# Rafae1130/qwen_inference_engine

Measured on AMD Instinct MI355X. Metric: decode tokens/s + prefill tok/s, Qwen2-7B bf16 batch=1, 1/2/4/8 MI355X, higher is better.
Workload: dtype bf16; 1 GPU; Qwen2-7B bf16 decode, batch=1, prompt=2048, gen=512; batch_per_gpu=1, batch=1, prompt=2048, gen=512, parallelism=single, graph=True, kv=contiguous

## Files before the change

include/qie/qie_engine.h:

```cpp
#ifndef QIE_ENGINE_H
#define QIE_ENGINE_H

#include "qie_types.h"
#include "qie_ops.h"

#ifdef __cplusplus
extern "C" {
#endif

typedef struct qie_engine qie_engine;
typedef struct qie_comm qie_comm;
typedef struct qie_batch qie_batch;
typedef struct qie_index qie_index;

int qie_index_load_meta(const char* meta_data_txt, qie_index** out);
int qie_index_synthetic(const qie_model_spec* spec, qie_index** out);
int qie_index_count(const qie_index* idx);
int qie_index_get(const qie_index* idx, int i, const char** name, const char** short_name,
                  int32_t* layer, int64_t* off0, int64_t* off1, int32_t* ndim, int64_t* shape4);
int64_t qie_index_total_bytes(const qie_index* idx);
int qie_index_write_meta(const qie_index* idx, const char* path);
void qie_index_destroy(qie_index* idx);

#define QIE_COMM_ID_BYTES 128
// ... 3 lines not shown
#define QIE_COMM_PEER_HANDLE_BYTES 128
int qie_comm_create_peer(int32_t world, int32_t rank, int32_t device, qie_comm** out, void* handle_out);
int qie_comm_peer_connect(qie_comm* c, const void* handles);
int qie_comm_create_peer_local(int32_t world, qie_comm** out);
int qie_comm_peer_error(const qie_comm* c, int32_t* err);
int qie_comm_peer_set_mode(qie_comm* c, int32_t tagged, int32_t push);
int qie_comm_allreduce_residual_bf16(qie_comm* c, const float* part, void* x, int64_t n, void* stream);
int qie_comm_time_exchange(qie_comm* c, const float* part, void* x, int64_t n, int32_t count, int32_t reps,
                           int32_t form, void* stream, float* us_out);
int qie_comm_rank(const qie_comm* c, int32_t* world, int32_t* rank);
int qie_comm_allreduce_sum_f32(qie_comm* c, float* buf, int64_t n, void* stream);
int qie_comm_allreduce_max_u64(qie_comm* c, uint64_t* buf, int64_t n, void* stream);
void qie_comm_destroy(qie_comm* c);

typedef struct qie_engine_opts {
    int32_t device;
    int32_t max_ctx;
    int32_t use_graph;
    int32_t tp_rank, tp_size;
    void* tp_comm;
    int32_t weight_fp8;
    int32_t comm_always;
    int32_t prefill_fp8;
    int32_t reserved[5];
} qie_engine_opts;

int qie_engine_create(const qie_model_spec* spec, const qie_engine_opts* opts, qie_engine** out);
int qie_engine_init_synthetic(qie_engine* e, uint64_t seed, float w_scale, float norm_scale,
                              float bias_scale);
int qie_engine_load_weights_bin(qie_engine* e, const char* weights_bin, const char* meta_data_txt,
                                int64_t chunk_bytes);
int qie_engine_set_weights(qie_engine* e, const qie_model_weights* w);
int qie_engine_weights(const qie_engine* e, qie_model_weights* out, const qie_layer_weights** layers);
int qie_engine_spec(const qie_engine* e, qie_model_spec* out);
void* qie_engine_stream(qie_engine* e);
int qie_engine_sync(qie_engine* e);
void qie_engine_destroy(qie_engine* e);

int qie_batch_create(qie_engine* e, int32_t batch, int32_t max_ctx, qie_batch** out);
void qie_batch_destroy(qie_batch* b);

int qie_batch_create_paged(qie_engine* e, int32_t batch, int32_t max_ctx, int32_t page_tokens,
                           int32_t n_pages, qie_batch** out);
int qie_batch_release(qie_batch* b, int32_t seq);
int qie_batch_page_stats(qie_batch* b, int32_t* free_pages, int32_t* pages_per_seq, int32_t* page_tokens);
int qie_batch_block_table(qie_batch* b, int32_t seq, int32_t* host_pages, int32_t n);

int qie_prefill(qie_batch* b, int32_t seq, const int32_t* ids, int32_t n, const qie_sampling* s,
                int32_t* next_id);
int qie_prefill_batch(qie_batch* b, int32_t seq0, int32_t n_seqs, const int32_t* ids, int32_t len,
                      const qie_sampling* s, int32_t* next_ids);
int qie_prefill_append(qie_batch* b, int32_t seq, const int32_t* ids, int32_t n, int32_t pos0,
                       const qie_sampling* s, int32_t* next_id);
int qie_decode_step(qie_batch* b, const qie_sampling* s, int32_t* next_ids);
int qie_decode(qie_batch* b, int32_t n_steps, const qie_sampling* s, int32_t* out_ids);
int qie_batch_logits(qie_batch* b, void* host_out);
int qie_batch_positions(qie_batch* b, int32_t* host_pos);
int qie_batch_history(qie_batch* b, int32_t seq, int32_t* host_ids, int32_t n);
int qie_batch_set_position(qie_batch* b, int32_t seq, int32_t pos, int32_t token);
int qie_batch_set_decode_mode(qie_batch* b, int32_t mode);
int qie_batch_decode_mode(const qie_batch* b);
int qie_batch_pk_trace(qie_batch* b, int32_t enable, uint64_t* host_out, int64_t n);
int qie_batch_dims(const qie_batch* b, int32_t* batch, int32_t* max_ctx);
int qie_batch_kv_cache(const qie_batch* b, int32_t seq, qie_kv_cache* out);
int qie_batch_reserve(qie_batch* b, int32_t seq, int32_t n_tokens);
int qie_engine_arena(const qie_engine* e, void** base, int64_t* bytes);
int qie_engine_rope_tables(const qie_engine* e, const float** rope_cos, const float** rope_sin,
                           int32_t* rows);
int qie_batch_time_kernel(qie_batch* b, int32_t which, int32_t iters, double* avg_us,
                          double* bytes);
int qie_batch_debug_step(qie_batch* b, const qie_sampling* smp, int32_t* next_ids, void* host_x);

#ifdef __cplusplus
}
#endif

#endif
```

qwen_inference_engine_amd/_lib.py:

```python
from __future__ import annotations

import ctypes as C
import os

_HERE = os.path.dirname(os.path.abspath(__file__))
LIB_PATH = os.environ.get("QIE_LIB") or os.path.join(_HERE, "lib", "libqie.so")

QIE_NUMERICS_REF = 0
QIE_NUMERICS_HF = 1
QIE_EPI_STORE = 0
QIE_EPI_RESIDUAL = 1
QIE_EPI_SWIGLU = 2
QIE_EPI_F32 = 3
QIE_LINEAR_FP8 = 1
QIE_LINEAR_TILE256 = 2
QIE_LINEAR_TILE128 = 4
QIE_LINEAR_STREAMK = 8
QIE_LINEAR_FP8_T16 = 16
QIE_LINEAR_ACT_FP8 = 32
QIE_ATTN_PREROPED = 0x100
QIE_COMM_ID_BYTES = 128
QIE_COMM_PEER_HANDLE_BYTES = 128


# ... 97 lines not shown
    ("qie_keys_to_ids", C.c_int, [_P, _I64, _P, _P]),
    ("qie_tensor_id", C.c_uint32, [C.c_char_p]),
    ("qie_synthetic_fill", C.c_int, [_P, _I64, _U32, _U64, _F, _F, _P]),
    ("qie_synthetic_fill_host", C.c_int, [_P, _I64, _U32, _U64, _F, _F]),
    ("qie_synthetic_fill_slice", C.c_int, [_P, _I64, _I64, _I64, _I64, _I64, _U32, _U64, _F, _F, _P]),
    ("qie_scale_rows_pow2", C.c_int, [_P, _I64, _I64, _I64, _I64, _I32, _P]),
    ("qie_fp8_weight_bytes", C.c_int64, [_I64, _I64]),
    ("qie_quantize_fp8", C.c_int, [_P, _I64, _I64, _P, _P]),
    ("qie_quantize_rows_fp8", C.c_int, [_P, _I64, _I64, _I64, _P, _I64, _P, _P]),
    ("qie_quantize_fp8_host", C.c_int, [_P, _I64, _I64, _P]),
    ("qie_dequantize_fp8", C.c_int, [_P, _I64, _I64, _P, _P]),
    ("qie_fp8_tile16", C.c_int, [_P, _I64, _I64, _P, _P]),
    ("qie_debug_fp8_decode", C.c_int, [_P]),
    ("qie_debug_fp8_decode_bf16", C.c_int, [_P]),
    ("qie_comm_unique_id", C.c_int, [_P]),
    ("qie_comm_create_rccl", C.c_int, [_P, _I32, _I32, _I32, C.POINTER(_P)]),
    ("qie_comm_create_local", C.c_int, [_I32, C.POINTER(_P)]),
    ("qie_comm_create_peer", C.c_int, [_I32, _I32, _I32, C.POINTER(_P), _P]),
    ("qie_comm_peer_connect", C.c_int, [_P, _P]),
    ("qie_comm_create_peer_local", C.c_int, [_I32, C.POINTER(_P)]),
    ("qie_comm_peer_error", C.c_int, [_P, _PI32]),
    ("qie_comm_allreduce_residual_bf16", C.c_int, [_P, _P, _P, _I64, _P]),
    ("qie_comm_peer_set_mode", C.c_int, [_P, _I32, _I32]),
    ("qie_comm_time_exchange", C.c_int, [_P, _P, _P, _I64, _I32, _I32, _I32, _P, C.POINTER(C.c_float)]),
    ("qie_comm_rank", C.c_int, [_P, _PI32, _PI32]),
    ("qie_comm_allreduce_sum_f32", C.c_int, [_P, _P, _I64, _P]),
    ("qie_comm_allreduce_max_u64", C.c_int, [_P, _P, _I64, _P]),
    ("qie_comm_destroy", None, [_P]),
    ("qie_index_load_meta", C.c_int, [C.c_char_p, C.POINTER(_P)]),
    ("qie_index_synthetic", C.c_int, [C.POINTER(ModelSpecC), C.POINTER(_P)]),
    ("qie_index_count", C.c_int, [_P]),
    ("qie_index_get", C.c_int, [_P, C.c_int, _PCC, _PCC, _PI32, _PI64, _PI64, _PI32, _PI64]),
    ("qie_index_total_bytes", C.c_int64, [_P]),
    ("qie_index_write_meta", C.c_int, [_P, C.c_char_p]),
    ("qie_index_destroy", None, [_P]),
    ("qie_engine_create", C.c_int, [C.POINTER(ModelSpecC), C.POINTER(EngineOptsC), C.POINTER(_P)]),
    ("qie_engine_init_synthetic", C.c_int, [_P, _U64, _F, _F, _F]),
    ("qie_engine_load_weights_bin", C.c_int, [_P, C.c_char_p, C.c_char_p, _I64]),
    ("qie_engine_set_weights", C.c_int, [_P, C.POINTER(ModelWeightsC)]),
    ("qie_engine_weights", C.c_int, [_P, C.POINTER(ModelWeightsC), C.POINTER(C.POINTER(LayerWeightsC))]),
    ("qie_engine_spec", C.c_int, [_P, C.POINTER(ModelSpecC)]),
    ("qie_engine_stream", _P, [_P]),
    ("qie_engine_sync", C.c_int, [_P]),
    ("qie_engine_destroy", None, [_P]),
    ("qie_batch_create", C.c_int, [_P, _I32, _I32, C.POINTER(_P)]),
    ("qie_batch_destroy", None, [_P]),
    ("qie_batch_create_paged", C.c_int, [_P, _I32, _I32, _I32, _I32, C.POINTER(_P)]),
    ("qie_batch_release", C.c_int, [_P, _I32]),
    ("qie_batch_page_stats", C.c_int, [_P, _PI32, _PI32, _PI32]),
    ("qie_batch_block_table", C.c_int, [_P, _I32, _PI32, _I32]),
    ("qie_prefill", C.c_int, [_P, _I32, _PI32, _I32, C.POINTER(SamplingC), _PI32]),
    ("qie_prefill_batch", C.c_int, [_P, _I32, _I32, _PI32, _I32, C.POINTER(SamplingC), _PI32]),
    ("qie_prefill_append", C.c_int, [_P, _I32, _PI32, _I32, _I32, C.POINTER(SamplingC), _PI32]),
    ("qie_decode_step", C.c_int, [_P, C.POINTER(SamplingC), _PI32]),
    ("qie_decode", C.c_int, [_P, _I32, C.POINTER(SamplingC), _PI32]),
    ("qie_batch_logits", C.c_int, [_P, _P]),
    ("qie_batch_positions", C.c_int, [_P, _PI32]),
    ("qie_batch_history", C.c_int, [_P, _I32, _PI32, _I32]),
    ("qie_batch_set_position", C.c_int, [_P, _I32, _I32, _I32]),
    ("qie_batch_dims", C.c_int, [_P, _PI32, _PI32]),
    ("qie_batch_set_decode_mode", C.c_int, [_P, _I32]),
    ("qie_batch_decode_mode", C.c_int, [_P]),
    ("qie_batch_pk_trace", C.c_int, [_P, _I32, _P, C.c_int64]),
    ("qie_batch_kv_cache", C.c_int, [_P, _I32, C.POINTER(KvCacheC)]),
    ("qie_batch_reserve", C.c_int, [_P, _I32, _I32]),
    ("qie_engine_arena", C.c_int, [_P, C.POINTER(_P), _PI64]),
    ("qie_engine_rope_tables", C.c_int, [_P, C.POINTER(_P), C.POINTER(_P), _PI32]),
    ("qie_batch_time_kernel", C.c_int, [_P, _I32, _I32, _PD, _PD]),
    ("qie_batch_debug_step", C.c_int, [_P, _P, _PI32, _P]),
]

_lib = None


class QieError(RuntimeError):
    pass


def load(path: str = LIB_PATH):
    global _lib
    if _lib is not None:
        return _lib
    if not os.path.exists(path):
        raise QieError(f"{path} not built; run __graft_entry__.build() or make -C "
                       f"qwen_inference_engine_amd/csrc")
    lib = C.CDLL(path)
    for name, res, args in SIGNATURES:
        fn = getattr(lib, name)
        fn.restype = res
        fn.argtypes = args
    _lib = lib
    return lib


def check(rc: int, what: str = "") -> None:
    if rc != 0:
        msg = _lib.qie_last_error().decode() if _lib is not None else ""
        raise QieError(f"{what} failed (rc={rc}): {msg}")
```

qwen_inference_engine_amd/csrc/engine.hip:

```cpp
#include "qie_common.hpp"
#include "linear_plan.hpp"
#include "../../include/qie/qie_engine.h"
#include "qie_index.hpp"
#include "qie_comm.hpp"

#include <chrono>
#include <cstring>
#include <fstream>
#include <vector>

namespace qie {
bool dec8_applies(const qie_linear_args* a);
int dec8_reserve(hipStream_t st);
bool persist_supported(const qie_model_spec& s, int B, int tp, bool fp8, bool paged, int ncu, const char** why);
size_t persist_attn_table_bytes(int n_layers);
int persist_attn_table(const qie_model_spec& s, const qie_layer_weights* h_layers, const void* qkv_scratch,
                       const int32_t* pos, const float* rope_cos, const float* rope_sin, const qie_kv_cache* cache,
                       void* dec_ws, void* d_attp, hipStream_t st);
int persist_decode_launch(const qie_model_spec& s, const qie_layer_weights* d_layers, const void* d_attp,
                          uint16_t* x_res, unsigned long long* granules, const unsigned* epoch, unsigned* err,
                          const int32_t* pos, int splits_target, unsigned long long* ts, hipStream_t st);
int64_t persist_granule_count(const qie_model_spec& s);
int persist_ts_slots();
}
// ... 540 lines not shown
    if (e->fp8_t16_head) a.flags |= QIE_LINEAR_FP8_T16;
    a.x = x; a.ldx = ldx;
    a.w[0] = e->w.lm_head; a.seg_rows[0] = Vl;
    a.M = M; a.K = s.hidden; a.N = Vl;
    a.y = b->logits + (int64_t)m0 * Vl; a.ldy = Vl;
    a.epilogue = QIE_EPI_STORE;
    a.norm_w = e->w.final_norm; a.norm_eps = s.rms_eps; a.numerics = s.numerics;
    QIE_TRY(prenorm(b, a, M));
    const bool greedy = is_greedy(smp);
    if (greedy) {
        a.argmax_keys = (uint64_t*)(b->d_keys + m0);
        a.key_col0 = e->sh.vocab0;
    }
    QIE_TRY(linear(&a, LinearExtras{}, st));
    if (greedy && use_comm(e)) QIE_TRY(e->comm->allreduce_max_u64((uint64_t*)(b->d_keys + m0), M, st));
    if (!greedy) {
        const uint16_t* lg = b->logits + (int64_t)m0 * Vl;
        if (use_comm(e)) {
            QIE_TRY(gather_logits(b, m0, M));
            lg = b->logits_full + (int64_t)m0 * s.vocab;
        }
        QIE_TRY(qie_sample(lg, M, s.vocab, s.vocab, smp, b->d_step + m0, b->d_ids + m0, b->samp_ws, st));
    }
    hipLaunchKernelGGL(finalize_kernel, dim3(M), dim3(256), 0, st, m0, greedy ? b->d_keys : nullptr,
                       b->d_ids, b->d_ids, b->d_pos, b->d_step, b->d_hist, b->max_ctx,
                       (const uint4*)e->w.embed, (uint4*)b->x_res, (int64_t)s.hidden / 8, s.vocab, rope_cur_args(b),
                       b->pk_mem ? pk_epoch_ptr(b) : nullptr);
    QIE_LAUNCH_CHECK();
    return 0;
}

static bool pk_on(const qie_batch* b) { return b->decode_mode == 1 && b->pk_mem && !b->dbg_x; }

static int pk_splits_target(const qie_batch* b) { (void)b; return 32; }

static int enqueue_layers_persistent(qie_batch* b) {
    qie_engine* e = b->e;
    return persist_decode_launch(e->spec, b->d_layers, b->d_attp, b->x_res, (unsigned long long*)b->pk_mem,
                                 pk_epoch_ptr(b), pk_epoch_ptr(b) + 1, b->d_pos, pk_splits_target(b), b->pk_ts,
                                 e->stream);
}

static int enqueue_decode(qie_batch* b, const qie_sampling* smp) {
    if (pk_on(b)) QIE_TRY(enqueue_layers_persistent(b));
    else
        for (int l = 0; l < b->e->spec.n_layers; l++) QIE_TRY(enqueue_layer_decode(b, l));
    return enqueue_head(b, b->x_res, b->e->spec.hidden, 0, b->B, smp);
}

static bool prefill_mx(const qie_engine* e) {
    return e->fp8 && e->opts.prefill_fp8;
}

static int64_t prefill_attn_ws_bytes(const qie_batch* b, int64_t n, bool extend) {
    const qie_model_spec& s = b->e->spec;
    if (extend) return qie_attention_extend_workspace_bytes(n, b->e->sh.nq, s.head_dim, b->max_ctx + b->run_pad);
    return qie_attention_workspace_bytes(n, b->e->sh.nq, s.head_dim, b->max_ctx);
}

static int ensure_prefill_scratch(qie_batch* b, int64_t n, bool extend) {
    if (n <= b->pf_rows) {
        const int64_t ws = prefill_attn_ws_bytes(b, n, extend);
        if (ws > b->pf_attn_ws_bytes) {
            hipFree(b->pf_attn_ws);
            b->pf_attn_ws = nullptr;
            b->pf_attn_ws_bytes = 0;
            QIE_TRY(dmalloc(&b->pf_attn_ws, (size_t)ws));
            b->pf_attn_ws_bytes = ws;
        }
        return 0;
    }
    const qie_model_spec& s = b->e->spec;
    const TpShard& sh = b->e->sh;
    const int64_t H = s.hidden, QD = (int64_t)sh.nq * s.head_dim, KD = (int64_t)sh.nkv * s.head_dim;
    void** olds[] = {(void**)&b->pf_x, (void**)&b->pf_hn, (void**)&b->pf_qkv, (void**)&b->pf_q, (void**)&b->pf_att,
                     (void**)&b->pf_h, (void**)&b->pf_pos, (void**)&b->pf_ids, &b->pf_attn_ws, (void**)&b->pf_part,
                     (void**)&b->pf_q8, (void**)&b->pf_e8};
    for (void** p : olds) {
        if (*p) hipFree(*p);
        *p = nullptr;
    }
    b->pf_rows = 0;
    if (use_comm(b->e)) QIE_TRY(dmalloc((void**)&b->pf_part, n * H * 4));
    QIE_TRY(dmalloc((void**)&b->pf_x, n * H * 2));
    QIE_TRY(dmalloc((void**)&b->pf_hn, n * H * 2));
    QIE_TRY(dmalloc((void**)&b->pf_qkv, n * (QD + 2 * KD) * 2));
    QIE_TRY(dmalloc((void**)&b->pf_q, n * QD * 2));
    QIE_TRY(dmalloc((void**)&b->pf_att, n * QD * 2));
    QIE_TRY(dmalloc((void**)&b->pf_h, n * (int64_t)sh.ffn * 2));
    if (prefill_mx(b->e)) {
        const int64_t kmax = std::max<int64_t>(std::max<int64_t>(H, QD), sh.ffn);
        QIE_TRY(dmalloc((void**)&b->pf_q8, n * kmax));
        QIE_TRY(dmalloc((void**)&b->pf_e8, std::max<int64_t>(n, 16)));
    }
    QIE_TRY(dmalloc((void**)&b->pf_pos, n * 4));
    QIE_TRY(dmalloc((void**)&b->pf_ids, n * 4));
    b->pf_attn_ws = nullptr;
    b->pf_attn_ws_bytes = 0;
    int64_t ws = prefill_attn_ws_bytes(b, n, extend);
    QIE_TRY(dmalloc(&b->pf_attn_ws, (size_t)ws));
    b->pf_attn_ws_bytes = ws;
    b->pf_rows = n;
    return 0;
}

static int pk_fail(unsigned w) {
    return fail(-8, "decode: the persistent decode step gave up on a hand-off wait (error word 0x%x: a CU never "
                    "published its part within the bound); outputs of this step are invalid", w);
}
static int pk_check(qie_batch* b) {
    if (!b->pk_mem) return 0;
    unsigned w = 0;
    QIE_HIP(hipMemcpyAsync(&w, pk_epoch_ptr(b) + 1, 4, hipMemcpyDeviceToHost, b->e->stream));
    QIE_HIP(hipStreamSynchronize(b->e->stream));
    return w ? pk_fail(w) : 0;
}

static int sync_ids(qie_batch* b, int32_t* next_ids) {
    if (!next_ids) return pk_check(b);
    qie_engine* e = b->e;
    QIE_HIP(hipMemcpyAsync(next_ids, b->d_ids, b->B * 4, hipMemcpyDeviceToHost, e->stream));
    const unsigned* ew = use_comm(e) ? e->comm->error_word() : nullptr;
    unsigned err = 0, pkw = 0;
    if (ew) QIE_HIP(hipMemcpyAsync(&err, ew, sizeof(err), hipMemcpyDeviceToHost, e->stream));
    if (b->pk_mem) QIE_HIP(hipMemcpyAsync(&pkw, pk_epoch_ptr(b) + 1, 4, hipMemcpyDeviceToHost, e->stream));
    QIE_HIP(hipStreamSynchronize(e->stream));
    if (pkw) return pk_fail(pkw);
    if (ew) {
        if (err) return fail(-7, "decode: tensor-parallel exchange failed on the device (error word %u: a peer rank "
                                 "did not arrive within the bounded wait); the communicator is unusable", err);
        return 0;
    }
    return comm_check(e, "decode");
}

}

extern "C" {

int qie_engine_create(const qie_model_spec* spec, const qie_engine_opts* opts, qie_engine** out) {
    QIE_REQUIRE(spec && out, "qie_engine_create: bad arguments");
    const qie_model_spec& s = *spec;
    QIE_REQUIRE(s.n_layers > 0 && s.hidden > 0 && s.n_heads > 0 && s.n_kv_heads > 0 && s.head_dim > 0 &&
                    s.ffn > 0 && s.vocab > 0 && s.n_heads % s.n_kv_heads == 0,
                "qie_engine_create: invalid model spec");
    QIE_REQUIRE(s.hidden % 8 == 0 && s.ffn % 8 == 0 && (s.head_dim == 64 || s.head_dim == 128),
                "qie_engine_create: hidden/ffn must be multiples of 8 and head_dim 64 or 128");
    qie_comm* comm = opts ? (qie_comm*)opts->tp_comm : nullptr;
    const int tp = comm ? comm->world : 1;
    TpShard probe;
    QIE_REQUIRE(shard_heads(s.n_heads, s.n_kv_heads, tp, 0, probe) && s.ffn % tp == 0 && (s.ffn / tp) % 8 == 0 &&
                    s.vocab % tp == 0,
// ... 416 lines not shown
    if (page_tokens == 0) page_tokens = 128;
    QIE_REQUIRE(page_tokens >= 128 && (page_tokens & (page_tokens - 1)) == 0,
                "qie_batch_create_paged: page_tokens %d must be a power of two >= 128", page_tokens);
    QIE_REQUIRE(n_pages >= 0, "qie_batch_create_paged: bad n_pages");
    QIE_REQUIRE(n_pages == 0 || n_pages >= 2, "qie_batch_create_paged: need the scratch page and one more");
    return batch_create(e, batch, max_ctx, page_tokens, n_pages, out);
}

int qie_batch_release(qie_batch* b, int32_t seq) {
    QIE_REQUIRE(b && seq >= 0 && seq < b->B, "qie_batch_release: bad arguments");
    drop_pages(b, seq);
    b->idle[seq] = 1;
    QIE_TRY(flush_table(b));
    qie_engine* e = b->e;
    hipLaunchKernelGGL(set_state_kernel, dim3(1), dim3(256), 0, e->stream, seq, 0, 0, 0, b->d_pos, b->d_step, b->d_hist,
                       b->max_ctx, (const uint4*)e->w.embed, (uint4*)b->x_res, (int64_t)e->spec.hidden / 8, 1, rope_cur_args(b));
    QIE_LAUNCH_CHECK();
    QIE_HIP(hipStreamSynchronize(e->stream));
    b->h_pos[seq] = 0;
    return 0;
}

int qie_batch_page_stats(qie_batch* b, int32_t* free_pages, int32_t* pages_per_seq, int32_t* page_tokens) {
    QIE_REQUIRE(b, "qie_batch_page_stats: null batch");
    if (free_pages) *free_pages = (int32_t)b->free_pages.size();
    if (pages_per_seq)
        for (int m = 0; m < b->B; m++) pages_per_seq[m] = b->d_table ? b->held[m] : 0;
    if (page_tokens) *page_tokens = b->page_tokens;
    return 0;
}

int qie_batch_block_table(qie_batch* b, int32_t seq, int32_t* host_pages, int32_t n) {
    QIE_REQUIRE(b && b->d_table && host_pages && seq >= 0 && seq < b->B && n >= 0 && n <= b->max_pages,
                "qie_batch_block_table: bad arguments (paged batch, n <= max_pages)");
    QIE_HIP(hipStreamSynchronize(b->e->stream));
    QIE_HIP(d2h(b->e, host_pages, b->d_table + (int64_t)seq * b->max_pages, (size_t)n * 4));
    return 0;
}

void qie_batch_destroy(qie_batch* b) {
    if (!b) return;
    if (b->e && b->e->stream) hipStreamSynchronize(b->e->stream);
    if (b->gexec) hipGraphExecDestroy(b->gexec);
    void* ps[] = {b->kc, b->vc, b->d_table, b->d_pos, b->d_rope_cur, b->d_step, b->d_hist, b->d_ids, b->d_keys, b->x_res, b->qkv, b->q,
                  b->att, b->h, b->logits, b->attn_ws, b->dec_ws, b->samp_ws, b->pf_x, b->pf_hn, b->pf_qkv, b->pf_q,
                  b->pf_att, b->pf_h, b->pf_pos, b->pf_ids, b->pf_attn_ws, b->part, b->logits_full,
                  b->gather_tmp, b->pf_part, b->xn, b->pf_q8, b->pf_e8, b->pk_mem, b->d_layers, b->d_attp, b->pk_ts};
    for (void* p : ps)
        if (p) hipFree(p);
    delete b;
}

static int prefill_rows(qie_batch* b, int seq0, int n_seqs, const int32_t* ids, int len, int pos0,
                        const qie_sampling* smp, int32_t* next_ids, const char* who) {
    QIE_REQUIRE(b && ids && len > 0 && n_seqs > 0 && seq0 >= 0 && seq0 + n_seqs <= b->B && pos0 >= 0,
                "%s: bad arguments", who);
    QIE_REQUIRE((int64_t)pos0 + len < b->max_ctx, "%s: %d tokens from position %d do not fit max_ctx %d", who, len,
                pos0, b->max_ctx);
    const bool append = pos0 > 0;
    qie_engine* e = b->e;
    const qie_model_spec& s = e->spec;
    if (append) {
        QIE_REQUIRE(n_seqs == 1, "%s: one sequence per call", who);
        QIE_REQUIRE(!b->idle[seq0], "%s: slot %d holds no live sequence", who, seq0);
        QIE_REQUIRE(pos0 <= b->h_pos[seq0], "%s: pos0 %d is past sequence %d's current position %d", who, pos0, seq0,
                    b->h_pos[seq0]);
        QIE_REQUIRE(!(e->fp8 && e->opts.prefill_fp8),
                    "%s: not available on a prefill_fp8 engine (block-scaled fp8 activations are defined for a "
                    "prefill from position 0 only: an append has no reference to be checked against)", who);
    }
    const int64_t n = (int64_t)n_seqs * len;
    QIE_REQUIRE(n <= INT32_MAX, "%s: %lld rows", who, (long long)n);
    for (int64_t i = 0; i < n; i++)
        QIE_REQUIRE(ids[i] >= 0 && ids[i] < s.vocab, "%s: token id %d out of range", who, ids[i]);
    hipStream_t st = e->stream;
    if (append && b->d_table) {
        const int64_t need = ((int64_t)pos0 + len + b->page_tokens - 1) / b->page_tokens - b->held[seq0];
        if (need > (int64_t)b->free_pages.size())
            return fail(-28, "%s: KV pool exhausted (%lld more pages needed for %d rows at position %d, %zu free)",
                        who, (long long)need, len, pos0, b->free_pages.size());
    }
    QIE_TRY(ensure_prefill_scratch(b, n, append));
    if (b->d_table && !append) {
        const int64_t need = ((int64_t)len + b->page_tokens - 1) / b->page_tokens * n_seqs;
        int64_t held = 0;
        for (int z = 0; z < n_seqs; z++) held += b->held[seq0 + z];
        QIE_REQUIRE(need <= (int64_t)b->free_pages.size() + held,
                    "%s: KV pool exhausted (%lld pages needed, %zu free + %lld held by slots %d..%d)", who,
                    (long long)need, b->free_pages.size(), (long long)held, seq0, seq0 + n_seqs - 1);
    }
    if (!append)
        for (int z = 0; z < n_seqs; z++) drop_pages(b, seq0 + z);
    for (int z = 0; z < n_seqs; z++) {
        QIE_TRY(ensure_pages(b, seq0 + z, (int64_t)pos0 + len));
        b->idle[seq0 + z] = 0;
    }
    QIE_TRY(flush_table(b));
    const TpShard& sh = e->sh;
    const int64_t H = s.hidden, hd = s.head_dim, QD = (int64_t)sh.nq * hd, KD = (int64_t)sh.nkv * hd;
    const int64_t QKVD = QD + 2 * KD, I = sh.ffn;
    QIE_HIP(hipMemcpyAsync(b->pf_ids, ids, (size_t)n * 4, hipMemcpyHostToDevice, st));
    hipLaunchKernelGGL(iota_kernel, dim3((unsigned)((n + 255) / 256)), dim3(256), 0, st, b->pf_pos, (int)n, len, pos0);
    hipLaunchKernelGGL(copy_ids_kernel, dim3((len + 255) / 256, n_seqs), dim3(256), 0, st, b->pf_ids,
                       b->d_hist + (int64_t)seq0 * b->max_ctx + pos0, len, (int64_t)b->max_ctx);
    QIE_TRY(qie_embedding(e->w.embed, b->pf_ids, b->pf_x, n, H, st));
    const qie_kv_cache cache = batch_cache(b, seq0);
    const bool pf16 = e->fp8 && !e->layers_pf.empty() && (n >= 256 || (e->fp8_t16 && n > 16));
    auto pf_base = [&]() {
        qie_linear_args a = lin_proj(e);
        if (pf16) a.flags &= ~(QIE_LINEAR_FP8 | QIE_LINEAR_FP8_T16);
        return a;
    };
    const bool mx = prefill_mx(e);
    auto attend = [&](int l) -> int {
        if (append)
            return qie_attention_extend(b->pf_q, n, b->pf_pos, len, &cache, l, sh.nq, b->pf_att, b->pf_attn_ws, st);
        return qie_attention(b->pf_q, n, b->pf_pos, len, &cache, l, sh.nq, b->pf_att, b->pf_attn_ws, st);
    };
    auto mx_in = [&](qie_linear_args& a, const uint16_t* x, int64_t K) -> int {
        QIE_TRY(qie_quantize_rows_fp8(x, K, n, K, b->pf_q8, K, b->pf_e8, st));
        a.x = b->pf_q8; a.ldx = K; a.x_exps = b->pf_e8;
        a.flags |= QIE_LINEAR_ACT_FP8;
        return 0;
    };
    for (int l = 0; l < s.n_layers; l++) {
        if (mx) {
            const qie_layer_weights& L = e->layers[l];
            QIE_TRY(qie_rmsnorm(b->pf_x, L.attn_norm, b->pf_hn, n, H, s.rms_eps, s.numerics, st));
            qie_linear_args a = lin_proj(e);
            QIE_TRY(mx_in(a, b->pf_hn, H));
            a.w[0] = L.wq; a.w[1] = L.wk; a.w[2] = L.wv;
            a.bias[0] = L.bq; a.bias[1] = L.bk; a.bias[2] = L.bv;
            a.seg_rows[0] = QD; a.seg_rows[1] = KD; a.seg_rows[2] = KD;
            a.M = n; a.K = H; a.N = QKVD; a.y = b->pf_qkv; a.ldy = QKVD; a.epilogue = QIE_EPI_STORE;
            QIE_TRY(qie_linear(&a, st));
            QIE_TRY(qie_qkv_post(b->pf_qkv, n, b->pf_pos, len, L.q_norm, L.k_norm, e->rope_cos, e->rope_sin, sh.nq,
                                 &cache, l, s.rms_eps, s.numerics, b->pf_q, st));
            QIE_TRY(attend(l));
            a = lin_proj(e);
            QIE_TRY(mx_in(a, b->pf_att, QD));
            a.w[0] = L.wo; a.seg_rows[0] = H;
            a.M = n; a.K = QD; a.N = H; a.ldy = H;
            QIE_TRY(row_parallel(b, a, b->pf_x, b->pf_part, n));
            QIE_TRY(qie_rmsnorm(b->pf_x, L.ffn_norm, b->pf_hn, n, H, s.rms_eps, s.numerics, st));
            a = lin_proj(e);
            QIE_TRY(mx_in(a, b->pf_hn, H));
            a.w[0] = L.w_gate; a.w[1] = L.w_up; a.seg_rows[0] = I; a.seg_rows[1] = I;
            a.M = n; a.K = H; a.N = I; a.y = b->pf_h; a.ldy = I; a.epilogue = QIE_EPI_SWIGLU;
            QIE_TRY(qie_linear(&a, st));
            a = lin_proj(e);
            QIE_TRY(mx_in(a, b->pf_h, I));
            a.w[0] = L.w_down; a.seg_rows[0] = H;
            a.M = n; a.K = I; a.N = H; a.ldy = H;
            QIE_TRY(row_parallel(b, a, b->pf_x, b->pf_part, n));
            continue;
        }
        const qie_layer_weights& L = pf16 ? e->layers_pf[l] : e->layers[l];
        QIE_TRY(qie_rmsnorm(b->pf_x, L.attn_norm, b->pf_hn, n, H, s.rms_eps, s.numerics, st));
        qie_linear_args a = pf_base();
        a.x = b->pf_hn; a.ldx = H;
        a.w[0] = L.wq; a.w[1] = L.wk; a.w[2] = L.wv;
        a.bias[0] = L.bq; a.bias[1] = L.bk; a.bias[2] = L.bv;
        a.seg_rows[0] = QD; a.seg_rows[1] = KD; a.seg_rows[2] = KD;
        a.M = n; a.K = H; a.N = QKVD; a.y = b->pf_qkv; a.ldy = QKVD; a.epilogue = QIE_EPI_STORE;
        QIE_TRY(qie_linear(&a, st));
        QIE_TRY(qie_qkv_post(b->pf_qkv, n, b->pf_pos, len, L.q_norm, L.k_norm, e->rope_cos, e->rope_sin, sh.nq,
                             &cache, l, s.rms_eps, s.numerics, b->pf_q, st));
        QIE_TRY(attend(l));
        a = pf_base();
        a.x = b->pf_att; a.ldx = QD; a.w[0] = L.wo; a.seg_rows[0] = H;
        a.M = n; a.K = QD; a.N = H; a.ldy = H;
        QIE_TRY(row_parallel(b, a, b->pf_x, b->pf_part, n));
        QIE_TRY(qie_rmsnorm(b->pf_x, L.ffn_norm, b->pf_hn, n, H, s.rms_eps, s.numerics, st));
        a = pf_base();
        a.x = b->pf_hn; a.ldx = H; a.w[0] = L.w_gate; a.w[1] = L.w_up; a.seg_rows[0] = I; a.seg_rows[1] = I;
        a.M = n; a.K = H; a.N = I; a.y = b->pf_h; a.ldy = I; a.epilogue = QIE_EPI_SWIGLU;
        QIE_TRY(qie_linear(&a, st));
        a = pf_base();
        a.x = b->pf_h; a.ldx = I; a.w[0] = L.w_down; a.seg_rows[0] = H;
        a.M = n; a.K = I; a.N = H; a.ldy = H;
        QIE_TRY(row_parallel(b, a, b->pf_x, b->pf_part, n));
    }
    for (int z = 0; z < n_seqs; z++) {
        hipLaunchKernelGGL(set_state_kernel, dim3(1), dim3(64), 0, st, seq0 + z, pos0 + len - 1, 0,
                           ids[(int64_t)z * len + len - 1], b->d_pos, b->d_step, b->d_hist, b->max_ctx,
                           (const uint4*)e->w.embed, (uint4*)b->x_res, (int64_t)H / 8, 0, rope_cur_args(b));
        QIE_LAUNCH_CHECK();
    }
    const uint16_t* last = b->pf_x + (int64_t)(len - 1) * H;
    if (n_seqs > 1) {
        QIE_HIP(hipMemcpy2DAsync(b->pf_hn, (size_t)H * 2, last, (size_t)len * H * 2, (size_t)H * 2, n_seqs,
                                 hipMemcpyDeviceToDevice, st));
        last = b->pf_hn;
    }
    QIE_TRY(enqueue_head(b, last, H, seq0, n_seqs, smp));
    for (int z = 0; z < n_seqs; z++) b->h_pos[seq0 + z] = pos0 + len;
    if (next_ids) {
        QIE_HIP(hipMemcpyAsync(next_ids, b->d_ids + seq0, (size_t)n_seqs * 4, hipMemcpyDeviceToHost, st));
        QIE_HIP(hipStreamSynchronize(st));
        QIE_TRY(comm_check(e, who));
    }
    return 0;
}

int qie_prefill(qie_batch* b, int32_t seq, const int32_t* ids, int32_t n, const qie_sampling* smp, int32_t* next_id) {
    return prefill_rows(b, seq, 1, ids, n, 0, smp, next_id, "qie_prefill");
}

int qie_prefill_append(qie_batch* b, int32_t seq, const int32_t* ids, int32_t n, int32_t pos0,
                       const qie_sampling* smp, int32_t* next_id) {
    QIE_REQUIRE(pos0 >= 1, "qie_prefill_append: pos0 must be >= 1 (a sequence starts with qie_prefill)");
    return prefill_rows(b, seq, 1, ids, n, pos0, smp, next_id, "qie_prefill_append");
}

int qie_prefill_batch(qie_batch* b, int32_t seq0, int32_t n_seqs, const int32_t* ids, int32_t len,
                      const qie_sampling* smp, int32_t* next_ids) {
    return prefill_rows(b, seq0, n_seqs, ids, len, 0, smp, next_ids, "qie_prefill_batch");
}

static bool same_sampling(const qie_sampling& a, const qie_sampling* b) {
    qie_sampling g{1, 0.f, 1.f, 0};
    const qie_sampling& bb = b ? *b : g;
    return a.top_k == bb.top_k && a.temperature == bb.temperature && a.top_p == bb.top_p && a.seed == bb.seed;
}

static int launch_step(qie_batch* b, const qie_sampling* smp) {
    qie_engine* e = b->e;
    if (!e->opts.use_graph) return enqueue_decode(b, smp);
    if (!b->graph_ok || !same_sampling(b->gs, smp)) {
        if (b->gexec) hipGraphExecDestroy(b->gexec);
        b->gexec = nullptr;
        b->graph_ok = false;
        hipGraph_t g = nullptr;
        QIE_HIP(hipStreamBeginCapture(e->stream, hipStreamCaptureModeThreadLocal));
        int rc = enqueue_decode(b, smp);
        hipError_t he = hipStreamEndCapture(e->stream, &g);
        if (rc) {
            if (g) hipGraphDestroy(g);
            return rc;
        }
        if (he != hipSuccess) return fail((int)he, "graph capture: %s", hipGetErrorString(he));
        if (dev_env("QIE_GRAPH_DUMP", 0)) {
            size_t n = 0;
            hipGraphGetNodes(g, nullptr, &n);
            std::vector<hipGraphNode_t> nodes(n);
            hipGraphGetNodes(g, nodes.data(), &n);
            size_t max_shm = 0;
            for (size_t i = 0; i < n; i++) {
                hipGraphNodeType t;
                hipGraphNodeGetType(nodes[i], &t);
                if (t == hipGraphNodeTypeKernel) {
                    hipKernelNodeParams kp{};
                    hipGraphKernelNodeGetParams(nodes[i], &kp);
                    max_shm = std::max(max_shm, (size_t)kp.sharedMemBytes);
                    fprintf(stderr, "graph node %zu: kernel %p grid %u,%u,%u block %u,%u,%u dyn_lds %u\n", i, kp.func,
                            kp.gridDim.x, kp.gridDim.y, kp.gridDim.z, kp.blockDim.x, kp.blockDim.y, kp.blockDim.z,
                            kp.sharedMemBytes);
                } else {
                    fprintf(stderr, "graph node %zu: type %d\n", i, (int)t);
                }
            }
            fprintf(stderr, "graph: %zu nodes, max dynamic LDS %zu B\n", n, max_shm);
        }
        he = hipGraphInstantiate(&b->gexec, g, nullptr, nullptr, 0);
        hipGraphDestroy(g);
// ... 389 lines not shown
```

qwen_inference_engine_amd/engine.py:

```python
from __future__ import annotations

import ctypes as C
import dataclasses
from typing import Dict, List, Optional, Sequence

import numpy as np

from . import _lib
from .spec import ModelSpec
from .weights import SynthParams

REF_PREFILL_SAMPLING = dict(top_k=50, temperature=1.0, seed=1234)
REF_DECODE_SAMPLING = dict(top_k=50, temperature=0.7, seed=1234)
REF_EOS = 151645


@dataclasses.dataclass
class Sampling:
    top_k: int = 1
    temperature: float = 1.0
    top_p: float = 1.0
    seed: int = 1234

    def to_c(self) -> _lib.SamplingC:
# ... 141 lines not shown
        _lib.check(self.lib.qie_engine_load_weights_bin(self.h, bin_path.encode(), meta_path.encode(),
                                                        chunk_bytes), "qie_engine_load_weights_bin")
        return self

    def set_weights(self, dev_ptrs: Dict[str, int], keepalive=None) -> "Engine":
        w, layers = weights_struct(self.spec, dev_ptrs)
        _lib.check(self.lib.qie_engine_set_weights(self.h, C.byref(w)), "qie_engine_set_weights")
        self._keep = (w, layers, keepalive)
        return self

    @property
    def stream(self) -> int:
        return self.lib.qie_engine_stream(self.h)

    def sync(self) -> None:
        _lib.check(self.lib.qie_engine_sync(self.h), "qie_engine_sync")

    def batch(self, batch: int = 1, max_ctx: Optional[int] = None, page_tokens: Optional[int] = None,
              n_pages: int = 0) -> "Batch":
        return Batch(self, batch, max_ctx or self.max_ctx, page_tokens, n_pages)

    def close(self) -> None:
        if getattr(self, "h", None):
            self.lib.qie_engine_destroy(self.h)
            self.h = None

    def __del__(self):
        try:
            self.close()
        except Exception:
            pass


class Batch:
    def __init__(self, engine: Engine, batch: int, max_ctx: int, page_tokens: Optional[int] = None,
                 n_pages: int = 0):
        self.e = engine
        self.lib = engine.lib
        self.B = batch
        self.max_ctx = max_ctx
        self.paged = page_tokens is not None
        h = C.c_void_p()
        if self.paged:
            _lib.check(self.lib.qie_batch_create_paged(engine.h, batch, max_ctx, page_tokens, n_pages, C.byref(h)),
                       "qie_batch_create_paged")
        else:
            _lib.check(self.lib.qie_batch_create(engine.h, batch, max_ctx, C.byref(h)), "qie_batch_create")
        self.h = h

    def prefill(self, seq: int, ids: Sequence[int], sampling: Sampling = GREEDY, chunk: Optional[int] = None) -> int:
        if chunk is not None:
            from .scheduler import prefill_chunks
            pieces = prefill_chunks(len(ids), chunk)
            tok = self.prefill(seq, ids[:pieces[0][1]], sampling)
            for off, n in pieces[1:]:
                tok = self.append(seq, ids[off:off + n], off, sampling)
            return tok
        arr = (C.c_int32 * len(ids))(*[int(i) for i in ids])
        out = C.c_int32(-1)
        sc = sampling.to_c()
        _lib.check(self.lib.qie_prefill(self.h, seq, arr, len(ids), C.byref(sc), C.byref(out)), "qie_prefill")
        return out.value

    def append(self, seq: int, ids: Sequence[int], pos0: Optional[int] = None, sampling: Sampling = GREEDY) -> int:
        if pos0 is None:
            pos0 = int(self.positions()[seq])
        arr = (C.c_int32 * len(ids))(*[int(i) for i in ids])
        out = C.c_int32(-1)
        sc = sampling.to_c()
        _lib.check(self.lib.qie_prefill_append(self.h, seq, arr, len(ids), int(pos0), C.byref(sc), C.byref(out)),
                   "qie_prefill_append")
        return out.value

    def prefill_batch(self, seq0: int, prompts: Sequence[Sequence[int]], sampling: Sampling = GREEDY) -> List[int]:
        n = len(prompts)
        length = len(prompts[0]) if n else 0
        if n == 0 or any(len(p) != length for p in prompts):
            raise ValueError("prefill_batch: needs one or more prompts of equal length")
        flat = np.ascontiguousarray(np.asarray(prompts, dtype=np.int32).reshape(-1))
        out = (C.c_int32 * n)()
        sc = sampling.to_c()
        _lib.check(self.lib.qie_prefill_batch(self.h, seq0, n, flat.ctypes.data_as(C.POINTER(C.c_int32)), length,
                                              C.byref(sc), out), "qie_prefill_batch")
        return list(out)

    def decode_step(self, sampling: Sampling = GREEDY) -> List[int]:
        out = (C.c_int32 * self.B)()
        sc = sampling.to_c()
        _lib.check(self.lib.qie_decode_step(self.h, C.byref(sc), out), "qie_decode_step")
        return list(out)

    def decode(self, n_steps: int, sampling: Sampling = GREEDY, want_ids: bool = True) -> Optional[np.ndarray]:
        out = np.zeros((max(n_steps, 1), self.B), dtype=np.int32)
        sc = sampling.to_c()
        ptr = out.ctypes.data_as(C.POINTER(C.c_int32)) if want_ids else None
        _lib.check(self.lib.qie_decode(self.h, n_steps, C.byref(sc), ptr), "qie_decode")
        return out[:n_steps] if want_ids else None

    def logits(self) -> np.ndarray:
        out = np.zeros((self.B, self.e.spec.vocab), dtype=np.uint16)
        _lib.check(self.lib.qie_batch_logits(self.h, out.ctypes.data), "qie_batch_logits")
        return out

    def positions(self) -> np.ndarray:
        out = np.zeros(self.B, dtype=np.int32)
        _lib.check(self.lib.qie_batch_positions(self.h, out.ctypes.data_as(C.POINTER(C.c_int32))),
                   "qie_batch_positions")
        return out

    def history(self, seq: int, n: int) -> np.ndarray:
        out = np.zeros(n, dtype=np.int32)
        _lib.check(self.lib.qie_batch_history(self.h, seq, out.ctypes.data_as(C.POINTER(C.c_int32)), n),
                   "qie_batch_history")
        return out

    def set_position(self, seq: int, pos: int, token: int) -> None:
        _lib.check(self.lib.qie_batch_set_position(self.h, seq, pos, token), "qie_batch_set_position")

    def release(self, seq: int) -> None:
        _lib.check(self.lib.qie_batch_release(self.h, seq), "qie_batch_release")

    def page_stats(self):
        free, pt = C.c_int32(), C.c_int32()
        per = np.zeros(self.B, dtype=np.int32)
        _lib.check(self.lib.qie_batch_page_stats(self.h, C.byref(free), per.ctypes.data_as(C.POINTER(C.c_int32)),
# ... 68 lines not shown
```

qwen_inference_engine_amd/scheduler.py:

```python
from __future__ import annotations

import collections
import dataclasses
from typing import Deque, Dict, List, Optional, Sequence

from .engine import GREEDY, Batch, Engine, Sampling


@dataclasses.dataclass
class Request:
    rid: int
    prompt: List[int]
    max_new_tokens: int
    stop_ids: tuple = ()
    tokens: List[int] = dataclasses.field(default_factory=list)
    logits: list = dataclasses.field(default_factory=list)
    slot: int = -1
    pages: int = 0
    done: bool = False
    chunks: list = dataclasses.field(default_factory=list)


def prefill_runs(admitted: Sequence[Request]) -> List[List[Request]]:
    runs: List[List[Request]] = []
# ... 30 lines not shown
        self.waiting: Deque[Request] = collections.deque()
        self.slots: List[Optional[Request]] = [None] * slots
        self.requests: Dict[int, Request] = {}
        self._next = 0

    def _pages(self, n_tokens: int) -> int:
        return -(-n_tokens // self.page_tokens)

    def submit(self, prompt: Sequence[int], max_new_tokens: int, stop_ids: Sequence[int] = ()) -> int:
        n = len(prompt)
        if n < 1 or max_new_tokens < 1 or n + max_new_tokens > self.max_ctx - 1:
            raise ValueError(f"request of {n} + {max_new_tokens} tokens does not fit max_ctx {self.max_ctx}")
        if self._pages(n + max_new_tokens) > self.budget + sum(r.pages for r in self.slots if r):
            raise ValueError("request larger than the whole page pool")
        r = Request(self._next, [int(t) for t in prompt], int(max_new_tokens), tuple(int(s) for s in stop_ids))
        self._next += 1
        self.requests[r.rid] = r
        self.waiting.append(r)
        return r.rid

    def _finish(self, r: Request) -> None:
        r.done = True
        self.batch.release(r.slot)
        self.slots[r.slot] = None
        self.budget += r.pages
        r.slot = -1

    def _emit(self, r: Request, tok: int, out: list, logits=None) -> None:
        r.tokens.append(tok)
        if self.keep_logits:
            r.logits.append((self.batch.logits() if logits is None else logits)[r.slot].copy())
        out.append((r.rid, tok))
        if len(r.tokens) >= r.max_new_tokens or tok in r.stop_ids:
            self._finish(r)

    def _admit(self, out: list) -> None:
        admitted: List[Request] = []
        while self.waiting:
            r = self.waiting[0]
            need = self._pages(len(r.prompt) + r.max_new_tokens)
            free_slot = next((i for i, s in enumerate(self.slots) if s is None), None)
            if free_slot is None or need > self.budget:
                break
            self.waiting.popleft()
            r.slot, r.pages = free_slot, need
            self.budget -= need
            self.slots[free_slot] = r
            admitted.append(r)
        first: Dict[int, int] = {}
        whole: List[Request] = []
        for r in admitted:
            pieces = prefill_chunks(len(r.prompt), self.prefill_chunk)
            if len(pieces) > 1:
                self.batch.prefill(r.slot, r.prompt[:pieces[0][1]], self.sampling)
                r.chunks = pieces[1:]
            else:
                whole.append(r)
        for run in prefill_runs(whole):
            if len(run) == 1:
                first[run[0].rid] = self.batch.prefill(run[0].slot, run[0].prompt, self.sampling)
            else:
                toks = self.batch.prefill_batch(run[0].slot, [r.prompt for r in run], self.sampling)
                first.update((r.rid, t) for r, t in zip(run, toks))
        lg = self.batch.logits() if self.keep_logits and whole else None
        for r in whole:
            self._emit(r, first[r.rid], out, lg)

    def _advance_chunks(self, out: list, fresh: set) -> None:
        for r in self.slots:
            if r is None or not r.chunks or r.rid in fresh:
                continue
            off, n = r.chunks.pop(0)
            tok = self.batch.append(r.slot, r.prompt[off:off + n], off, self.sampling)
            if not r.chunks:
                self._emit(r, tok, out)

    def step(self) -> List[tuple]:
        out: List[tuple] = []
        before = {r.rid for r in self.slots if r is not None}
        self._admit(out)
        self._advance_chunks(out, {r.rid for r in self.slots if r is not None} - before)
        if any(s is not None for s in self.slots):
            live = list(self.slots)
            ids = self.batch.decode_step(self.sampling)
            lg = self.batch.logits() if self.keep_logits else None
            for i, r in enumerate(live):
                if r is not None and not r.done and not r.chunks:
                    self._emit(r, int(ids[i]), out, lg)
        return out

    def idle(self) -> bool:
        return not self.waiting and all(s is None for s in self.slots)

    def run(self) -> Dict[int, List[int]]:
        while not self.idle():
            self.step()
        return {rid: r.tokens for rid, r in self.requests.items()}

    def close(self) -> None:
        self.batch.close()
```

Baseline: 367.6 tokens/s.

## Compute last-layer prefill tail only for final rows; add logit-free feed for chunks

In prefill, the last layer now stops after QKV/KV-cache write, and attention, o-proj and MLP for that layer run only on the final token row(s) of each sequence before the LM head. This skips the full-length last-layer attention and FFN whose outputs are discarded except for the last token. A new qie_prefill_feed entry point runs intermediate chunks without the head or sampling and sets state as if positioned after the chunk. The attention workspace sizing is extended to cover the tail call. It adds a separate code path for the tail, with its own fp8/bf16 weight selection.

```diff
diff --git a/include/qie/qie_engine.h b/include/qie/qie_engine.h
--- a/include/qie/qie_engine.h
+++ b/include/qie/qie_engine.h
@@ -79,6 +79,7 @@
                       const qie_sampling* s, int32_t* next_ids);
 int qie_prefill_append(qie_batch* b, int32_t seq, const int32_t* ids, int32_t n, int32_t pos0,
                        const qie_sampling* s, int32_t* next_id);
+int qie_prefill_feed(qie_batch* b, int32_t seq, const int32_t* ids, int32_t n, int32_t pos0);
 int qie_decode_step(qie_batch* b, const qie_sampling* s, int32_t* next_ids);
 int qie_decode(qie_batch* b, int32_t n_steps, const qie_sampling* s, int32_t* out_ids);
 int qie_batch_logits(qie_batch* b, void* host_out);
diff --git a/qwen_inference_engine_amd/_lib.py b/qwen_inference_engine_amd/_lib.py
--- a/qwen_inference_engine_amd/_lib.py
+++ b/qwen_inference_engine_amd/_lib.py
@@ -173,6 +173,7 @@
     ("qie_prefill", C.c_int, [_P, _I32, _PI32, _I32, C.POINTER(SamplingC), _PI32]),
     ("qie_prefill_batch", C.c_int, [_P, _I32, _I32, _PI32, _I32, C.POINTER(SamplingC), _PI32]),
     ("qie_prefill_append", C.c_int, [_P, _I32, _PI32, _I32, _I32, C.POINTER(SamplingC), _PI32]),
+    ("qie_prefill_feed", C.c_int, [_P, _I32, _PI32, _I32, _I32]),
     ("qie_decode_step", C.c_int, [_P, C.POINTER(SamplingC), _PI32]),
     ("qie_decode", C.c_int, [_P, _I32, C.POINTER(SamplingC), _PI32]),
     ("qie_batch_logits", C.c_int, [_P, _P]),
diff --git a/qwen_inference_engine_amd/csrc/engine.hip b/qwen_inference_engine_amd/csrc/engine.hip
--- a/qwen_inference_engine_amd/csrc/engine.hip
+++ b/qwen_inference_engine_amd/csrc/engine.hip
@@ -616,15 +616,17 @@
     return e->fp8 && e->opts.prefill_fp8;
 }
 
-static int64_t prefill_attn_ws_bytes(const qie_batch* b, int64_t n, bool extend) {
+static int64_t prefill_attn_ws_bytes(const qie_batch* b, int64_t n, int64_t n_seqs, bool extend) {
     const qie_model_spec& s = b->e->spec;
-    if (extend) return qie_attention_extend_workspace_bytes(n, b->e->sh.nq, s.head_dim, b->max_ctx + b->run_pad);
-    return qie_attention_workspace_bytes(n, b->e->sh.nq, s.head_dim, b->max_ctx);
-}
-
-static int ensure_prefill_scratch(qie_batch* b, int64_t n, bool extend) {
+    const int64_t tail = qie_attention_workspace_bytes(n_seqs, b->e->sh.nq, s.head_dim, b->max_ctx);
+    if (extend)
+        return std::max(tail, qie_attention_extend_workspace_bytes(n, b->e->sh.nq, s.head_dim, b->max_ctx + b->run_pad));
+    return std::max(tail, qie_attention_workspace_bytes(n, b->e->sh.nq, s.head_dim, b->max_ctx));
+}
+
+static int ensure_prefill_scratch(qie_batch* b, int64_t n, int64_t n_seqs, bool extend) {
     if (n <= b->pf_rows) {
-        const int64_t ws = prefill_attn_ws_bytes(b, n, extend);
+        const int64_t ws = prefill_attn_ws_bytes(b, n, n_seqs, extend);
         if (ws > b->pf_attn_ws_bytes) {
             hipFree(b->pf_attn_ws);
             b->pf_attn_ws = nullptr;
@@ -661,7 +663,7 @@
     QIE_TRY(dmalloc((void**)&b->pf_ids, n * 4));
     b->pf_attn_ws = nullptr;
     b->pf_attn_ws_bytes = 0;
-    int64_t ws = prefill_attn_ws_bytes(b, n, extend);
+    int64_t ws = prefill_attn_ws_bytes(b, n, n_seqs, extend);
     QIE_TRY(dmalloc(&b->pf_attn_ws, (size_t)ws));
     b->pf_attn_ws_bytes = ws;
     b->pf_rows = n;
@@ -1184,7 +1186,7 @@
 }
 
 static int prefill_rows(qie_batch* b, int seq0, int n_seqs, const int32_t* ids, int len, int pos0,
-                        const qie_sampling* smp, int32_t* next_ids, const char* who) {
+                        const qie_sampling* smp, int32_t* next_ids, const char* who, bool feed = false) {
     QIE_REQUIRE(b && ids && len > 0 && n_seqs > 0 && seq0 >= 0 && seq0 + n_seqs <= b->B && pos0 >= 0,
                 "%s: bad arguments", who);
     QIE_REQUIRE((int64_t)pos0 + len < b->max_ctx, "%s: %d tokens from position %d do not fit max_ctx %d", who, len,
@@ -1212,7 +1214,7 @@
             return fail(-28, "%s: KV pool exhausted (%lld more pages needed for %d rows at position %d, %zu free)",
                         who, (long long)need, len, pos0, b->free_pages.size());
     }
-    QIE_TRY(ensure_prefill_scratch(b, n, append));
+    QIE_TRY(ensure_prefill_scratch(b, n, n_seqs, append));
     if (b->d_table && !append) {
         const int64_t need = ((int64_t)len + b->page_tokens - 1) / b->page_tokens * n_seqs;
         int64_t held = 0;
@@ -1237,20 +1239,25 @@
                        b->d_hist + (int64_t)seq0 * b->max_ctx + pos0, len, (int64_t)b->max_ctx);
     QIE_TRY(qie_embedding(e->w.embed, b->pf_ids, b->pf_x, n, H, st));
     const qie_kv_cache cache = batch_cache(b, seq0);
-    const bool pf16 = e->fp8 && !e->layers_pf.empty() && (n >= 256 || (e->fp8_t16 && n > 16));
-    auto pf_base = [&]() {
+    auto on_pf16 = [&](int64_t rows) {
+        return e->fp8 && !e->layers_pf.empty() && (rows >= 256 || (e->fp8_t16 && rows > 16));
+    };
+    const bool pf16 = on_pf16(n);
+    auto base = [&](bool bf16_copy) {
         qie_linear_args a = lin_proj(e);
-        if (pf16) a.flags &= ~(QIE_LINEAR_FP8 | QIE_LINEAR_FP8_T16);
+        if (bf16_copy) a.flags &= ~(QIE_LINEAR_FP8 | QIE_LINEAR_FP8_T16);
         return a;
     };
+    auto pf_base = [&]() { return base(pf16); };
     const bool mx = prefill_mx(e);
     auto attend = [&](int l) -> int {
         if (append)
             return qie_attention_extend(b->pf_q, n, b->pf_pos, len, &cache, l, sh.nq, b->pf_att, b->pf_attn_ws, st);
         return qie_attention(b->pf_q, n, b->pf_pos, len, &cache, l, sh.nq, b->pf_att, b->pf_attn_ws, st);
     };
+    int64_t mx_rows = n;
     auto mx_in = [&](qie_linear_args& a, const uint16_t* x, int64_t K) -> int {
-        QIE_TRY(qie_quantize_rows_fp8(x, K, n, K, b->pf_q8, K, b->pf_e8, st));
+        QIE_TRY(qie_quantize_rows_fp8(x, K, mx_rows, K, b->pf_q8, K, b->pf_e8, st));
         a.x = b->pf_q8; a.ldx = K; a.x_exps = b->pf_e8;
         a.flags |= QIE_LINEAR_ACT_FP8;
         return 0;
@@ -1268,6 +1275,7 @@
             QIE_TRY(qie_linear(&a, st));
             QIE_TRY(qie_qkv_post(b->pf_qkv, n, b->pf_pos, len, L.q_norm, L.k_norm, e->rope_cos, e->rope_sin, sh.nq,
                                  &cache, l, s.rms_eps, s.numerics, b->pf_q, st));
+            if (l == s.n_layers - 1) break;
             QIE_TRY(attend(l));
             a = lin_proj(e);
             QIE_TRY(mx_in(a, b->pf_att, QD));
@@ -1298,6 +1306,7 @@
         QIE_TRY(qie_linear(&a, st));
         QIE_TRY(qie_qkv_post(b->pf_qkv, n, b->pf_pos, len, L.q_norm, L.k_norm, e->rope_cos, e->rope_sin, sh.nq,
                              &cache, l, s.rms_eps, s.numerics, b->pf_q, st));
+        if (l == s.n_layers - 1) break;
         QIE_TRY(attend(l));
         a = pf_base();
         a.x = b->pf_att; a.ldx = QD; a.w[0] = L.wo; a.seg_rows[0] = H;
@@ -1313,19 +1322,79 @@
         a.M = n; a.K = I; a.N = H; a.ldy = H;
         QIE_TRY(row_parallel(b, a, b->pf_x, b->pf_part, n));
     }
+    if (feed) {
+        for (int z = 0; z < n_seqs; z++) {
+            hipLaunchKernelGGL(set_state_kernel, dim3(1), dim3(64), 0, st, seq0 + z, pos0 + len, 1,
+                               ids[(int64_t)z * len + len - 1], b->d_pos, b->d_step, b->d_hist, b->max_ctx,
+                               (const uint4*)e->w.embed, (uint4*)b->x_res, (int64_t)H / 8, 1, rope_cur_args(b));
+            QIE_LAUNCH_CHECK();
+            b->h_pos[seq0 + z] = pos0 + len;
+        }
+        QIE_HIP(hipStreamSynchronize(st));
+        return comm_check(e, who);
+    }
     for (int z = 0; z < n_seqs; z++) {
         hipLaunchKernelGGL(set_state_kernel, dim3(1), dim3(64), 0, st, seq0 + z, pos0 + len - 1, 0,
                            ids[(int64_t)z * len + len - 1], b->d_pos, b->d_step, b->d_hist, b->max_ctx,
                            (const uint4*)e->w.embed, (uint4*)b->x_res, (int64_t)H / 8, 0, rope_cur_args(b));
         QIE_LAUNCH_CHECK();
     }
-    const uint16_t* last = b->pf_x + (int64_t)(len - 1) * H;
+    const int lt = s.n_layers - 1;
+    const int64_t T = n_seqs;
+    uint16_t* tq = b->pf_q + (int64_t)(len - 1) * QD;
+    uint16_t* tx = b->pf_x + (int64_t)(len - 1) * H;
     if (n_seqs > 1) {
-        QIE_HIP(hipMemcpy2DAsync(b->pf_hn, (size_t)H * 2, last, (size_t)len * H * 2, (size_t)H * 2, n_seqs,
+        QIE_HIP(hipMemcpy2DAsync(b->pf_qkv, (size_t)QD * 2, tq, (size_t)len * QD * 2, (size_t)QD * 2, n_seqs,
                                  hipMemcpyDeviceToDevice, st));
-        last = b->pf_hn;
-    }
-    QIE_TRY(enqueue_head(b, last, H, seq0, n_seqs, smp));
+        QIE_HIP(hipMemcpy2DAsync(b->pf_hn, (size_t)H * 2, tx, (size_t)len * H * 2, (size_t)H * 2, n_seqs,
+                                 hipMemcpyDeviceToDevice, st));
+        tq = b->pf_qkv;
+        tx = b->pf_hn;
+    }
+    QIE_TRY(qie_attention(tq, T, b->d_pos + seq0, 1, &cache, lt, sh.nq, b->pf_att, b->pf_attn_ws, st));
+    if (mx) {
+        const qie_layer_weights& L = e->layers[lt];
+        mx_rows = T;
+        qie_linear_args a = lin_proj(e);
+        QIE_TRY(mx_in(a, b->pf_att, QD));
+        a.w[0] = L.wo; a.seg_rows[0] = H;
+        a.M = T; a.K = QD; a.N = H; a.ldy = H;
+        QIE_TRY(row_parallel(b, a, tx, b->pf_part, T));
+        QIE_TRY(qie_rmsnorm(tx, L.ffn_norm, b->xn, T, H, s.rms_eps, s.numerics, st));
+        a = lin_proj(e);
+        QIE_TRY(mx_in(a, b->xn, H));
+        a.w[0] = L.w_gate; a.w[1] = L.w_up; a.seg_rows[0] = I; a.seg_rows[1] = I;
+        a.M = T; a.K = H; a.N = I; a.y = b->pf_h; a.ldy = I; a.epilogue = QIE_EPI_SWIGLU;
+        QIE_TRY(qie_linear(&a, st));
+        a = lin_proj(e);
+        QIE_TRY(mx_in(a, b->pf_h, I));
+        a.w[0] = L.w_down; a.seg_rows[0] = H;
+        a.M = T; a.K = I; a.N = H; a.ldy = H;
+        QIE_TRY(row_parallel(b, a, tx, b->pf_part, T));
+    } else {
+        const bool t16 = on_pf16(T);
+        const qie_layer_weights& L = t16 ? e->layers_pf[lt] : e->layers[lt];
+        qie_linear_args a = base(t16);
+        a.x = b->pf_att; a.ldx = QD; a.w[0] = L.wo; a.seg_rows[0] = H;
+        a.M = T; a.K = QD; a.N = H; a.ldy = H;
+        QIE_TRY(row_parallel(b, a, tx, b->pf_part, T));
+        a = base(t16);
+        a.x = tx; a.ldx = H; a.w[0] = L.w_gate; a.w[1] = L.w_up; a.seg_rows[0] = I; a.seg_rows[1] = I;
+        a.M = T; a.K = H; a.N = I; a.y = b->pf_h; a.ldy = I; a.epilogue = QIE_EPI_SWIGLU;
+        if (T <= 16) {
+            a.norm_w = L.ffn_norm; a.norm_eps = s.rms_eps; a.numerics = s.numerics;
+            QIE_TRY(prenorm(b, a, T));
+        } else {
+            QIE_TRY(qie_rmsnorm(tx, L.ffn_norm, b->xn, T, H, s.rms_eps, s.numerics, st));
+            a.x = b->xn;
+        }
+        QIE_TRY(linear(&a, LinearExtras{}, st));
+        a = base(t16);
+        a.x = b->pf_h; a.ldx = I; a.w[0] = L.w_down; a.seg_rows[0] = H;
+        a.M = T; a.K = I; a.N = H; a.ldy = H;
+        QIE_TRY(row_parallel(b, a, tx, b->pf_part, T));
+    }
+    QIE_TRY(enqueue_head(b, tx, H, seq0, n_seqs, smp));
     for (int z = 0; z < n_seqs; z++) b->h_pos[seq0 + z] = pos0 + len;
     if (next_ids) {
         QIE_HIP(hipMemcpyAsync(next_ids, b->d_ids + seq0, (size_t)n_seqs * 4, hipMemcpyDeviceToHost, st));
@@ -1343,6 +1412,10 @@
                        const qie_sampling* smp, int32_t* next_id) {
     QIE_REQUIRE(pos0 >= 1, "qie_prefill_append: pos0 must be >= 1 (a sequence starts with qie_prefill)");
     return prefill_rows(b, seq, 1, ids, n, pos0, smp, next_id, "qie_prefill_append");
+}
+
+int qie_prefill_feed(qie_batch* b, int32_t seq, const int32_t* ids, int32_t n, int32_t pos0) {
+    return prefill_rows(b, seq, 1, ids, n, pos0, nullptr, nullptr, "qie_prefill_feed", true);
 }
 
 int qie_prefill_batch(qie_batch* b, int32_t seq0, int32_t n_seqs, const int32_t* ids, int32_t len,
diff --git a/qwen_inference_engine_amd/engine.py b/qwen_inference_engine_amd/engine.py
--- a/qwen_inference_engine_amd/engine.py
+++ b/qwen_inference_engine_amd/engine.py
@@ -217,10 +217,10 @@
         if chunk is not None:
             from .scheduler import prefill_chunks
             pieces = prefill_chunks(len(ids), chunk)
-            tok = self.prefill(seq, ids[:pieces[0][1]], sampling)
-            for off, n in pieces[1:]:
-                tok = self.append(seq, ids[off:off + n], off, sampling)
-            return tok
+            for off, n in pieces[:-1]:
+                self.feed(seq, ids[off:off + n], off)
+            off, n = pieces[-1]
+            return self.append(seq, ids[off:], off, sampling) if off else self.prefill(seq, ids, sampling)
         arr = (C.c_int32 * len(ids))(*[int(i) for i in ids])
         out = C.c_int32(-1)
         sc = sampling.to_c()
@@ -236,6 +236,10 @@
         _lib.check(self.lib.qie_prefill_append(self.h, seq, arr, len(ids), int(pos0), C.byref(sc), C.byref(out)),
                    "qie_prefill_append")
         return out.value
+
+    def feed(self, seq: int, ids: Sequence[int], pos0: int = 0) -> None:
+        arr = (C.c_int32 * len(ids))(*[int(i) for i in ids])
+        _lib.check(self.lib.qie_prefill_feed(self.h, seq, arr, len(ids), int(pos0)), "qie_prefill_feed")
 
     def prefill_batch(self, seq0: int, prompts: Sequence[Sequence[int]], sampling: Sampling = GREEDY) -> List[int]:
         n = len(prompts)
diff --git a/qwen_inference_engine_amd/scheduler.py b/qwen_inference_engine_amd/scheduler.py
--- a/qwen_inference_engine_amd/scheduler.py
+++ b/qwen_inference_engine_amd/scheduler.py
@@ -106,7 +106,7 @@
         for r in admitted:
             pieces = prefill_chunks(len(r.prompt), self.prefill_chunk)
             if len(pieces) > 1:
-                self.batch.prefill(r.slot, r.prompt[:pieces[0][1]], self.sampling)
+                self.batch.feed(r.slot, r.prompt[:pieces[0][1]], 0)
                 r.chunks = pieces[1:]
             else:
                 whole.append(r)
@@ -125,9 +125,10 @@
             if r is None or not r.chunks or r.rid in fresh:
                 continue
             off, n = r.chunks.pop(0)
-            tok = self.batch.append(r.slot, r.prompt[off:off + n], off, self.sampling)
-            if not r.chunks:
-                self._emit(r, tok, out)
+            if r.chunks:
+                self.batch.feed(r.slot, r.prompt[off:off + n], off)
+            else:
+                self._emit(r, self.batch.append(r.slot, r.prompt[off:off + n], off, self.sampling), out)
 
     def step(self) -> List[tuple]:
         out: List[tuple] = []
```

New measurement: 367.3 tokens/s. No clear change (-0.1%).
